# Zilong-Li/BaseVarC

Hardware: AMD Instinct MI355X
Metric: sites/sec at N=1e6 samples; achieved HBM GB/s vs roofline (higher is better)
Workload: dtype f64

## Files before the change

basevarc_amd/csrc/bvc_context.hip:

```cpp
#include <cmath>
#include <cstdlib>
#include <cstring>
#include <mutex>
#include <new>

#include "bvc_ctx.h"

hipError_t sync_streams(bvc_ctx *ctx)
{
    hipError_t first = hipSuccess;
    for (hipStream_t s : streams_of(ctx)) {
        const hipError_t e = hipStreamSynchronize(s);
        if (first == hipSuccess) first = e;
    }
    for (bool &p : ctx->em_pending) p = false;
    return first;
}

int drain_on_error(bvc_ctx *ctx, int code)
{
    (void)sync_streams(ctx);
    (void)hipGetLastError();
    return code;
}
// ... 71 lines not shown
namespace {
std::mutex g_pinned_mu;
std::vector<std::pair<const char *, size_t>> g_pinned;
}

bool in_pinned(const void *p, size_t n)
{
    std::lock_guard<std::mutex> g(g_pinned_mu);
    const char *c = static_cast<const char *>(p);
    for (auto const &r : g_pinned)
        if (c >= r.first && c + n <= r.first + r.second) return true;
    return false;
}

namespace {
struct Knob {
    const char *key, *env;
    int lo, hi, step, dflt;
    int LaunchState::*member;
    bool takes(int v) const { return v >= lo && v <= hi && (v - lo) % step == 0; }
};
const Knob kKnobs[] = {
    {"em_waves_per_cu", "BVC_EM_WAVES_PER_CU", 0, 32, 1, 0, &LaunchState::em_waves_per_cu},
    {"em_wpb", "BVC_EM_WPB", 1, 4, 3, 4, &LaunchState::em_wpb},
    {"hist_split", "BVC_HIST_SPLIT", 0, 64, 1, 0, &LaunchState::hist_split},
    {"group_pipe", "BVC_GROUP_PIPE", 0, 1, 1, 1, &LaunchState::group_pipe},
    {"group_copies_log2", "BVC_GROUP_LOG2C", -1, 5, 1, -1, &LaunchState::group_log2c},
    {"group_big_lds", "BVC_GROUP_BIG_LDS", 0, 1, 1, 1, &LaunchState::group_big_lds},
    {"group_h16", "BVC_GROUP_H16", 0, 1, 1, 0, &LaunchState::group_h16},
    {"em_streams", "BVC_EM_STREAMS", 0, 3, 1, 0, &LaunchState::em_streams},
    {"em_engine", "BVC_EM_ENGINE", 0, 1, 1, 0, &LaunchState::em_engine},
    {"em_tiny_regions", "BVC_EM_TINY_REGIONS", 0, 1, 1, 0, &LaunchState::em_tiny_regions},
    {"em_prune", "BVC_EM_PRUNE", 0, 1, 1, 1, &LaunchState::em_prune},
    {"bgzf_codes", "BVC_BGZF_CODES", 0, 1, 1, 0, &LaunchState::bgzf_codes},
    {"bgzf_parse", "BVC_BGZF_PARSE", 0, 1, 1, 0, &LaunchState::bgzf_parse},
    {"bgzf_cuts", "BVC_BGZF_CUTS", 0, 1, 1, 0, &LaunchState::bgzf_cuts},
    {"csr_scatter_max", "BVC_CSR_SCATTER_MAX", 0, 1 << 30, 1, 64, &LaunchState::csr_scatter_max},
    {"stats_copies_log2", "BVC_STATS_LOG2C", 0, kStatsMaxLog2c, 1, 2, &LaunchState::stats_log2c},
    {"host_chunk_kib", nullptr, 1, 1 << 21, 1, 1 << 19, &LaunchState::host_chunk_kib},
};
}

extern "C" {

const char *bvc_version(void) { return "libbvc 0.3.0 (gfx950)"; }

int bvc_device_count(void)
{
    int n = 0;
    if (hipGetDeviceCount(&n) != hipSuccess) { (void)hipGetLastError(); return 0; }
    int ok = 0;
    for (int d = 0; d < n; ++d) {
        hipDeviceProp_t p;
        if (hipGetDeviceProperties(&p, d) == hipSuccess && std::strncmp(p.gcnArchName, "gfx950", 6) == 0) ++ok;
    }
    return ok;
}

static int env_int(const char *name, int lo, int hi, int dflt)
{
    const char *e = getenv(name);
    if (!e) return dflt;
    const int v = atoi(e);
    return (v >= lo && v <= hi) ? v : dflt;
}

// ... 241 lines not shown
```

basevarc_amd/csrc/bvc_internal.h:

```cpp
#pragma once
#include <hip/hip_runtime.h>
#include <stdint.h>

#include <vector>

#include "../../include/bvc.h"

struct bvc_bam_site_tally;

namespace bvc {

struct LaunchState {
    int n_cu = 256;
    int em_waves_per_cu = 0;
    int em_wpb = 4;
    int hist_split = 0;
    int host_chunk_kib = 1 << 19;
    int em_streams = 0;
    int group_pipe = 1;
    int group_log2c = -1;
    int group_big_lds = 1;
    int group_h16 = 0;
    int em_engine = 0;
    int em_tiny_regions = 0;
    int csr_scatter_max = 64;
    int em_prune = 1;
    int stats_log2c = 2;
    int bgzf_codes = 0;
    int bgzf_parse = 0;
    int bgzf_cuts = 0;
    int dbg_levels = 0;
    mutable uint32_t em_epoch = 0;
    struct RaisedLds { const void *kernel; size_t bytes; };
    mutable std::vector<RaisedLds> lds_raised;
};

inline size_t round256(size_t n) { return (n + 255) / 256 * 256; }

struct Layout {
    uintptr_t base = 0;
    size_t at = 0;
    template <class T> T *take(size_t count, size_t pad = 0)
    {
        T *p = reinterpret_cast<T *>(base + at);
        at += round256(count * sizeof(T) + pad);
        return p;
    }
};

hipError_t raise_lds(const LaunchState &st, const void *kernel, size_t bytes);

struct QualLut {
    double a[128];
    double e[128];
    double e_empty;
    double log_e[128];
    double log_a[128];
};

hipError_t launch_hist_dense(LaunchState &st, hipStream_t stream, int64_t n_sites, int64_t n_samples, int64_t row_stride,
                             const int8_t *bases, const int8_t *quals, const uint8_t *group_of_sample,
                             int n_groups, uint32_t *counts, int split, int64_t *group_scratch = nullptr,
                             uint8_t *hist_of_sample = nullptr);
constexpr int kGroupScratchWords = BVC_MAX_GROUPS + 4;
inline size_t group_redo_offset(int64_t n_samples) { return ((size_t)n_samples + 255) & ~(size_t)255; }
inline size_t group_labels_bytes(int64_t n_samples, int64_t n_sites) { return group_redo_offset(n_samples) + (size_t)n_sites + 256; }
int choose_hist_split(const LaunchState &st, int64_t n_sites, int64_t n_samples);

hipError_t launch_hist_packed(LaunchState &st, hipStream_t stream, int64_t n_sites, int64_t n_samples, int64_t row_stride,
                              const uint8_t *packed, uint32_t *counts, int split);
hipError_t launch_hist_packed_groups(LaunchState &st, hipStream_t stream, int64_t n_sites, int64_t n_samples,
                                     int64_t row_stride, const uint8_t *packed, const uint8_t *group_of_sample, int n_groups,
                                     uint32_t *counts, int64_t *group_scratch, uint8_t *hist_of_sample);
hipError_t launch_pack_dense(hipStream_t stream, int64_t n_sites, int64_t n_samples, int64_t stride_in, const int8_t *bases,
                             const int8_t *quals, int64_t stride_out, uint8_t *packed, unsigned long long *bad);

hipError_t launch_stream_read(hipStream_t stream, const void *src, int64_t bytes, uint32_t *sink);

hipError_t launch_hist_csr(LaunchState &st, hipStream_t stream, int64_t n_sites, const int64_t *offsets,
                           const int8_t *bases, const int8_t *quals, uint32_t *counts);

inline bool uses_item_engine(const LaunchState &st, double min_af) { return st.em_engine != 1 && min_af > 0.0; }
hipError_t launch_lrt(const LaunchState &st, hipStream_t stream, int64_t n_sites, const uint32_t *counts,
                      int64_t hist_stride, const int8_t *ref_base, double min_af, const QualLut *lut,
                      const int8_t *comb, const uint8_t *n_comb, bvc_site_result *results, bool shared = false,
                      int shared_waves_per_cu = 0,
                      void *scratch = nullptr);

size_t em_items_scratch_bytes(int64_t n_sites);
hipError_t launch_lrt_items(const LaunchState &st, hipStream_t stream, int64_t n_sites, int n_groups,
                            const uint32_t *counts, int64_t hist_stride, const int8_t *ref_base, double min_af,
                            const QualLut *lut, const int8_t *comb, const uint8_t *n_comb, bvc_site_result *results,
                            void *scratch, const uint8_t **taken_out, bool shared = false);

hipError_t launch_lrt_groups(const LaunchState &st, hipStream_t stream, int64_t n_sites, int n_groups,
                             const uint32_t *grp_counts, const int8_t *ref_base, double min_af, const QualLut *lut,
                             const bvc_site_result *overall, bvc_group_result *grp_results, bool shared = false,
                             int shared_waves_per_cu = 0, void *scratch = nullptr);
size_t em_group_scratch_bytes(int64_t n_sites, int n_groups);
constexpr int kGroupSharedWavesPerCu = 8;

hipError_t launch_sum_groups(hipStream_t stream, int64_t n_sites, int n_hist, const uint32_t *grp_counts,
                             uint32_t *counts);

hipError_t launch_synth_dense(hipStream_t stream, uint64_t seed, int64_t site0, int64_t n_sites,
                              int64_t n_samples, int64_t row_stride, uint32_t cov_thr16,
                              int8_t *bases, int8_t *quals, int8_t *ref_base);

struct PileupTile {
    const uint8_t *text = nullptr;
    bool bin = false;
    const uint32_t *line_start = nullptr;
    const int32_t *sample0 = nullptr, *n_in_batch = nullptr;
    int32_t n_batches = 0, n_pos = 0;
    int32_t line_stride = 0;
    const int32_t *n_pos_dev = nullptr;
    int64_t n_lines_cap = 0;
    uint32_t *line_words = nullptr;
    uint32_t *status = nullptr;
    int64_t *entry_off = nullptr, *obs_off = nullptr, *totals = nullptr;
    bvc_pileup_entry *entries = nullptr;
    int32_t *samples = nullptr;
    int8_t *obs_base = nullptr, *obs_qual = nullptr;
    const uint8_t *group_of_sample = nullptr;
    int64_t n_samples = 0;
    int32_t n_groups = 0;
    uint8_t *obs_label = nullptr;
    int32_t *tally = nullptr;
    bvc_pileup_indel *indels = nullptr;
    uint32_t indel_cap = 0;
};
struct bvc_pileup_region { uint32_t start, len, left_src, left_len; };
hipError_t launch_region_carry(hipStream_t stream, const uint8_t *old_text, uint8_t *text, const bvc_pileup_region *regions, int32_t n_batches);
hipError_t launch_region_index(hipStream_t stream, const PileupTile &P, const bvc_pileup_region *regions, const uint32_t *seg_base,
                               int64_t n_segments, uint32_t *seg_nl, int32_t *lines, int32_t max_pos);
hipError_t launch_region_ends(hipStream_t stream, const PileupTile &P, uint32_t *ends);
// ... 126 lines not shown
```

basevarc_amd/csrc/bvc_lrt.hip:

```cpp
#include "bvc_ctx.h"

namespace {

int em_stream_count(const bvc_ctx *ctx, int by_default) { return ctx->ls.em_streams > 0 ? ctx->ls.em_streams : by_default; }

hipStream_t em_stream(bvc_ctx *ctx, int by_default)
{
    const int n = em_stream_count(ctx, by_default);
    const int k = (int)(ctx->side_flip++ % (unsigned)n);
    return k == 0 ? ctx->side : (k == 1 ? ctx->side_b : ctx->side_c);
}

int em_scratch_for(bvc_ctx *ctx, int slot, int64_t n_sites, double min_af, void **out, int n_groups = 0)
{
    *out = nullptr;
    if (!uses_item_engine(ctx->ls, min_af)) return BVC_OK;
    const size_t need = n_groups > 0 ? em_group_scratch_bytes(n_sites, n_groups) : em_items_scratch_bytes(n_sites);
    DevBuf &buf = n_groups > 0 ? ctx->d_emg[slot] : ctx->d_em[slot];
    const int rc = ensure_joined(ctx, buf, need);
    if (rc != BVC_OK) return rc;
    *out = buf.p;
    return BVC_OK;
}

// ... 144 lines not shown
        if (rc != BVC_OK) return rc;
        if (n_rows == 1) d.rows[1] = d.rows[0];
    }
    return run_chunks(ctx, n_sites, chunk,
        [&](int set, int64_t s0, int64_t ns) -> int {
            const DenseSet &d = sets[set];
            const size_t bytes = n_samples ? (size_t)(ns - 1) * (size_t)row_stride + (size_t)n_samples : 0;
            if (n_groups > 0 && s0 < 2 * chunk && n_samples)
                BVC_HIP(ctx, hipMemcpyAsync(d.labels, labels, (size_t)n_samples, hipMemcpyHostToDevice, ctx->copy));
            for (int a = 0; a < n_rows && bytes; ++a)
                BVC_HIP(ctx, hipMemcpyAsync(d.rows[a], rows[a] + s0 * row_stride, bytes, hipMemcpyHostToDevice, ctx->copy));
            BVC_HIP(ctx, hipMemcpyAsync(d.ref, ref_base + s0, (size_t)ns, hipMemcpyHostToDevice, ctx->copy));
            return BVC_OK;
        },
        [&](int set, int64_t s0, int64_t ns, bool download) -> int {
            const DenseSet &d = sets[set];
            if (!download) {
                int rc = device(ns, d);
                return rc == BVC_OK ? join_side(ctx) : rc;
            }
            BVC_HIP(ctx, hipMemcpyAsync(results + s0, d.res, (size_t)ns * sizeof(bvc_site_result), hipMemcpyDeviceToHost, ctx->stream));
            if (n_groups > 0)
                BVC_HIP(ctx, hipMemcpyAsync(grp_results + s0 * n_groups, d.gres, (size_t)ns * n_groups * sizeof(bvc_group_result),
                                            hipMemcpyDeviceToHost, ctx->stream));
            return BVC_OK;
        });
}

template <class Stage1>
int run_group_stages(bvc_ctx *ctx, int64_t ns, int n_groups, bool long_rows, Stage1 stage1, const int8_t *r, double min_af,
                     bvc_site_result *res, bvc_group_result *gres, const uint32_t *grp_in = nullptr)
{
    return run_stages(ctx, ns, n_groups, false, min_af, 2, stage1, [&](hipStream_t s2, const RingSlot &slot) -> int {
        BVC_HIP(ctx, launch_sum_groups(s2, ns, n_groups + 1, slot.grp, slot.counts));
        const bool shared = ctx->overlap && long_rows;
        const int per_launch = kGroupSharedWavesPerCu / em_stream_count(ctx, 2) > 2 ? kGroupSharedWavesPerCu / em_stream_count(ctx, 2) : 2;
        BVC_HIP(ctx, launch_lrt(ctx->ls, s2, ns, slot.counts, BVC_NCLASS, r, min_af, ctx->d_lut, nullptr, nullptr, res, shared, per_launch,
                                slot.em));
        BVC_HIP(ctx, launch_lrt_groups(ctx->ls, s2, ns, n_groups, slot.grp, r, min_af, ctx->d_lut, res, gres, shared, per_launch, slot.emg));
        return BVC_OK;
    }, grp_in);
}

int run_csr_groups_device(bvc_ctx *ctx, int64_t n_sites, const int64_t *offsets, const int8_t *bases, const int8_t *quals,
                          const int32_t *sample_of_obs, const int8_t *ref_base, double min_af, const uint8_t *group_of_sample,
                          int64_t n_samples, int32_t n_groups, bvc_site_result *results, bvc_group_result *grp_results)
{
    return run_group_stages(ctx, n_sites, n_groups, false,
                            [&](uint32_t *gp) {
                                return launch_hist_csr_groups(ctx->ls, ctx->stream, n_sites, offsets, bases, quals, sample_of_obs,
                                                              group_of_sample, n_samples, n_groups, gp);
                            },
                            ref_base, min_af, results, grp_results);
}


struct ObsArray { const void *host; size_t elem; void *dev; };

template <class Device>
int run_csr_groups_host(bvc_ctx *ctx, int64_t n_sites, const int64_t *offsets, const int8_t *ref_base, const uint8_t *group_of_sample,
                        int64_t n_samples, ObsArray *arrays, int n_arrays, int32_t n_groups, bvc_site_result *results,
                        bvc_group_result *grp_results, Device device)
{
    const size_t total = (size_t)offsets[n_sites];
    int64_t *d_o; int8_t *d_r; uint8_t *d_g; bvc_site_result *d_res; bvc_group_result *d_gres;
    int rc = carve(ctx, ctx->d_stage[0], 256, [&](Layout &L) {
        d_o = L.take<int64_t>((size_t)n_sites + 1);
// ... 476 lines not shown
```

basevarc_amd/csrc/em_items.hip:

```cpp
#include <algorithm>

#include "bvc_device.h"
#include "bvc_internal.h"
#include "em_common.h"

namespace bvc {
namespace {



constexpr int kTiny = 8, kNarrow = 32, kWide = 48;
template <int CPB> constexpr int site_table_bytes() { return 4 * CPB * 5; }

constexpr int kEmptyQ = 128;

struct FitItem {
    int32_t site;
    uint8_t base[4];
    double f0[4];
    double e_excl;
    double inv_n;
    double ll_excl;
};
static_assert(sizeof(FitItem) == 64, "FitItem layout");
// ... 690 lines not shown
        finished = true;
    }
    S.sets = sets; S.n_emit = (int8_t)n_emit; S.p_deepest = (int8_t)p_deepest;
    int want[kLists];
    count_wanted(sets, n_emit, want);
    if (lane == 0) {
        if (finished) {
            store_record(results + site, S, (int)ref_base[ref_index(site, n_groups)], S.n, S.blist);
            S.state = 2;
        }
        R.site[ls] = S;
        R.want[ls][0] = want[0]; R.want[ls][1] = want[1];
    }
}

struct RegionArgs {
    int64_t n_sites;
    int n_groups;
    const uint32_t *counts;
    int64_t hist_stride;
    const QualLut *lut;
    const int8_t *ref_base;
    double min_af;
    const int8_t *comb;
    const uint8_t *n_comb;
    uint8_t *taken;
    bvc_site_result *results;
    uint32_t *kind_epoch;
    uint32_t epoch;
    int dbg_levels;
    int tiny_regions;
    int prune;
    int64_t region0;
};

__device__ __forceinline__ void wave_sync()
{
    __builtin_amdgcn_fence(__ATOMIC_RELEASE, "workgroup");
    __builtin_amdgcn_wave_barrier();
    __builtin_amdgcn_fence(__ATOMIC_ACQUIRE, "workgroup");
}

__device__ __forceinline__ void load_counts(uint32_t (&c)[8], const uint32_t *__restrict__ counts, int64_t hist_stride, int64_t site,
                                            int n_groups, int lane)
{
    const uint32_t *hist = counts + hist_index(site, n_groups) * hist_stride + (lane >> 4) * 128 + (lane & 15);
#pragma unroll
    for (int lvl = 0; lvl < 8; ++lvl) c[lvl] = hist[16 * lvl];
}

template <int TEAM, class RegionT>
__device__ __forceinline__ void team_sync(RegionT &R, uint32_t &phase, int lane)
{
    if (TEAM == 1) { wave_sync(); return; }
    __builtin_amdgcn_fence(__ATOMIC_RELEASE, "workgroup");
    __builtin_amdgcn_wave_barrier();
    phase += TEAM;
    if (lane == 0) {
        __hip_atomic_fetch_add(&R.arrive, 1u, __ATOMIC_RELEASE, __HIP_MEMORY_SCOPE_WORKGROUP);
        while (__hip_atomic_load(&R.arrive, __ATOMIC_ACQUIRE, __HIP_MEMORY_SCOPE_WORKGROUP) - phase > 0x7FFFFFFFu) __builtin_amdgcn_s_sleep(1);
    }
    __builtin_amdgcn_wave_barrier();
    __builtin_amdgcn_fence(__ATOMIC_ACQUIRE, "workgroup");
}

template <int CPB, int TEAM>
__device__ __forceinline__ void region_body(Region<CPB> *regions, const RegionArgs &A)
{
    const int wave = __builtin_amdgcn_readfirstlane((int)(threadIdx.x >> 6));
    const int teams = (int)(blockDim.x >> 6) / TEAM;
    const int member = wave % TEAM;
    const int lane = threadIdx.x & (kWave - 1);
    Region<CPB> &R = regions[wave / TEAM];
    const int64_t n_sites = A.n_sites;
    const int64_t n_regions = (n_sites + kRegionSites - 1) / kRegionSites;
    if (CPB == kWide && A.kind_epoch[1] != A.epoch) return;
    if (CPB == kTiny && A.kind_epoch[0] != A.epoch) return;
    uint32_t phase = 0;
    if (TEAM > 1) {
        if (member == 0 && lane == 0) R.arrive = 0u;
        __syncthreads();
    }
    const int64_t region = A.region0 + (int64_t)blockIdx.x * teams + wave / TEAM;
    for (bool first = true; region < n_regions && first; first = false) {
        const int64_t site0 = region * kRegionSites;
        if (member == 0 && lane == 0) { R.need = 0; R.next_slot = 0; }
        if (TEAM > 1) team_sync<TEAM>(R, phase, lane);
        int need = 0;
        uint32_t cnext[8];
        if (site0 + member < n_sites) load_counts(cnext, A.counts, A.hist_stride, site0 + member, A.n_groups, lane);
#pragma unroll 1
        for (int ls = member; ls < kRegionSites; ls += TEAM) {
            uint32_t c8[8];
#pragma unroll
            for (int k = 0; k < 8; ++k) c8[k] = cnext[k];
            if (ls + TEAM < kRegionSites && site0 + ls + TEAM < n_sites) load_counts(cnext, A.counts, A.hist_stride, site0 + ls + TEAM, A.n_groups, lane);
            if (site0 + ls < n_sites) {
                need = max(need, site_classes<CPB>(R, ls, lane, site0 + ls, c8, A.lut, A.min_af, A.comb, A.n_comb, A.taken));
            } else if (lane == 0) {
                R.site[ls].state = 2; R.site[ls].n_emit = 0;
                R.want[ls][0] = 0; R.want[ls][1] = 0;
            }
        }
        if (TEAM > 1) {
            if (lane == 0) atomicMax(&R.need, need);
            team_sync<TEAM>(R, phase, lane);
            need = R.need;
        } else {
            wave_sync();
        }
        const int kind = (A.tiny_regions && need <= kTiny) ? kTiny : (need <= kNarrow ? kNarrow : kWide);
        if (CPB == kNarrow && kind != kNarrow && member == 0 && lane == 0) A.kind_epoch[kind == kWide ? 1 : 0] = A.epoch;
        if (kind != CPB) {
            if (TEAM > 1) team_sync<TEAM>(R, phase, lane);
            continue;
        }
        if (member == 0 && lane < kRegionSites && R.site[lane].state == 3) {
            const int64_t site = site0 + lane;
            store_record(A.results + site, R.site[lane], (int)A.ref_base[ref_index(site, A.n_groups)], R.site[lane].n,
                         R.site[lane].blist);
            R.site[lane].state = 2;
        }
        team_sync<TEAM>(R, phase, lane);
        for (int round = 0; round < kRounds && round < (A.dbg_levels >> 1); ++round) {
            int cnt[kLists] = {0, 0};
#pragma unroll
            for (int w = 0; w < kRegionSites; ++w) {
#pragma unroll
                for (int l = 0; l < kLists; ++l) cnt[l] += R.want[w][l];
// ... 24 lines not shown
            team_sync<TEAM>(R, phase, lane);
            if (TEAM > 1 && member == 0 && lane == 0) R.next_slot = 0;
            if (round + 1 == (A.dbg_levels >> 1) && (A.dbg_levels & 1)) break;
            int my = lane;
            asm volatile("" : "+v"(my));
            if (member == 0 && my < kRegionSites && site0 + my < n_sites)
                site_decide(R, my, 0, site0 + my, A.n_groups, A.prune, A.ref_base, A.results);
            team_sync<TEAM>(R, phase, lane);
        }
        team_sync<TEAM>(R, phase, lane);
    }
}

#define BVC_OCCUPANCY(n) BVC_WAVES_PER_EU(n, n)
#ifdef BVC_RCP_CHUNK
#define BVC_REGION_WAVES_PER_EU 4
#else
#define BVC_REGION_WAVES_PER_EU 3
#endif
constexpr int kMaxRegionWaves = 4;
#ifndef BVC_REGION_TEAM
#define BVC_REGION_TEAM 2
#endif
constexpr int kTeam = BVC_REGION_TEAM;

template <int CPB>
__global__ __launch_bounds__(64 * kMaxRegionWaves) BVC_OCCUPANCY(CPB == kWide ? 2 : BVC_REGION_WAVES_PER_EU) void region_kernel(RegionArgs A)
{
    BVC_POISON_LDS();
    extern __shared__ __attribute__((aligned(16))) unsigned char region_lds[];
    region_body<CPB, kTeam>(reinterpret_cast<Region<CPB> *>(region_lds), A);
}

}

#ifdef BVC_CHECK_LDS
BVC_DEFINE_DEBUG_READER(debug_read_items)
#endif

struct ItemScratch {
    uint8_t *taken;
    uint32_t *kind_epoch;
};

static ItemScratch item_scratch(Layout &L, int64_t n_sites)
{
    const size_t start = L.at;
    ItemScratch s;
    s.taken = L.take<uint8_t>((size_t)n_sites);
    s.kind_epoch = L.take<uint32_t>(0);
    L.at = start + (size_t)n_sites + 256 + 64;
    return s;
}

size_t em_items_scratch_bytes(int64_t n_sites)
{
    Layout size;
    item_scratch(size, n_sites);
    return size.at;
}

hipError_t launch_lrt_items(const LaunchState &st, hipStream_t stream, int64_t n_sites, int n_groups,
                            const uint32_t *counts, int64_t hist_stride, const int8_t *ref_base, double min_af,
                            const QualLut *lut, const int8_t *comb, const uint8_t *n_comb, bvc_site_result *results,
                            void *scratch, const uint8_t **taken_out, bool shared)
{
    Layout slices{reinterpret_cast<uintptr_t>(scratch)};
    const ItemScratch scr = item_scratch(slices, n_sites);
    uint8_t *taken = scr.taken;
    const int64_t regions = (n_sites + kRegionSites - 1) / kRegionSites;
    int per_cu = 0;
    if (st.em_waves_per_cu > 0) per_cu = st.em_waves_per_cu;
    else if (shared) per_cu = 4;
    constexpr int kMaxTeams = kMaxRegionWaves / kTeam;
    int teams;
    int64_t wgs, per_launch;
    if (per_cu > 0) {
        const int want_teams = std::max(1, per_cu / kTeam);
        teams = std::min(want_teams, kMaxTeams);
        wgs = (regions + teams - 1) / teams;
        per_launch = (int64_t)st.n_cu * ((want_teams + teams - 1) / teams);
    } else {
        teams = (int)std::min<int64_t>(kMaxTeams, std::max<int64_t>(1, (regions + st.n_cu - 1) / st.n_cu));
        wgs = (regions + teams - 1) / teams;
        per_launch = wgs;
    }
    RegionArgs A;
    A.n_sites = n_sites; A.n_groups = n_groups; A.counts = counts; A.hist_stride = hist_stride; A.lut = lut;
    A.ref_base = ref_base; A.min_af = min_af; A.comb = comb; A.n_comb = n_comb; A.taken = taken; A.results = results;
    A.kind_epoch = scr.kind_epoch;
    A.epoch = ++st.em_epoch;
    if (A.epoch == 0) A.epoch = ++st.em_epoch;
    A.dbg_levels = st.dbg_levels > 0 ? st.dbg_levels : 2 * kRounds;
    A.tiny_regions = st.em_tiny_regions;
    A.prune = st.em_prune;
    A.region0 = 0;
    const hipError_t e = raise_lds(st, reinterpret_cast<const void *>(region_kernel<kWide>), kMaxTeams * sizeof(Region<kWide>));
    if (e != hipSuccess) return e;
    const dim3 block(64 * teams * kTeam);
    auto sequence = [&](auto kernel, size_t lds_per_team) {
        for (int64_t w0 = 0; w0 < wgs; w0 += per_launch) {
            A.region0 = w0 * teams;
            hipLaunchKernelGGL(kernel, dim3((unsigned)std::min(per_launch, wgs - w0)), block, teams * lds_per_team, stream, A);
        }
        A.region0 = 0;
    };
    sequence(region_kernel<kNarrow>, sizeof(Region<kNarrow>));
    if (st.em_tiny_regions) sequence(region_kernel<kTiny>, sizeof(Region<kTiny>));
    sequence(region_kernel<kWide>, sizeof(Region<kWide>));
    *taken_out = taken;
    return hipGetLastError();
}

}
```

basevarc_amd/csrc/em_kernel.hip:

```cpp
#include "bvc_device.h"
#include "bvc_internal.h"
#include "em_common.h"

namespace bvc {
namespace {

template <int NS>
struct Slots {
    double n[NS];
    double e[NS];
    double d[NS];
    double yp[NS];
};

struct Freq {
    double fb;
};

constexpr int kDppRor8 = 0x128;
constexpr int kDppRowBcast15 = 0x142;
template <int L> constexpr int dpp_newbcast() { return 0x150 + L; }

struct PassOut {
    double ex_own;
    bool converged;
};


template <int NS, int NA = NS>
__device__ __forceinline__ PassOut em_pass(Slots<NS> &S, const Freq f, double inv_n, int lane)
{
    static_assert(NA >= 1 && NA <= NS, "active slots");
// ... 376 lines not shown
            bvc_group_result r;
            for (int j = 0; j < 4; ++j) r.depth[j] = o.depth[j];
            for (int j = 0; j < 6; ++j) r.pad[j] = 0;
            r.ran = o.depth_total > 0 ? 1 : 0;
            r.present = 0;
#pragma unroll
            for (int i = 0; i < 3; ++i) {
                double af = 0.0;
                if (r.ran && i < ov.n_alt) {
#pragma unroll
                    for (int tt = 0; tt < 3; ++tt)
                        if (tt < o.n_alt && o.alt_base[tt] == ov.alt_base[i]) { af = o.af[tt]; r.present |= (uint8_t)(1u << i); }
                }
                r.af[i] = af;
            }
            grp_results[site * n_groups + g] = r;
        }
        wave_lds_sync<WPB>();
    }
}

__global__ void var_qual_kernel(int64_t n_sites, bvc_site_result *__restrict__ results)
{
    BVC_POISON_LDS();
    const int64_t s = (int64_t)blockIdx.x * blockDim.x + threadIdx.x;
    if (s >= n_sites) return;
    if (!results[s].called || results[s].var_qual != kVarQualPending) return;
    const double p = kf_gammaq_dev(0.5, results[s].chi / 2.0);
    double vq = (p != 0.0) ? -10 * log10(p) : 10000.0;
    if (vq == 0) vq = 0.0;
    results[s].var_qual = vq;
}

__global__ void sum_groups_kernel(int64_t total, int n_hist, const uint32_t *__restrict__ grp_counts,
                                  uint32_t *__restrict__ counts)
{
    BVC_POISON_LDS();
    const int64_t i = (int64_t)blockIdx.x * blockDim.x + threadIdx.x;
    if (i >= total) return;
    const int64_t site = i / BVC_NCLASS;
    const int key = (int)(i % BVC_NCLASS);
    uint32_t s = 0;
    for (int h = 0; h < n_hist; ++h) s += grp_counts[(site * n_hist + h) * BVC_NCLASS + key];
    counts[i] = s;
}

__global__ void group_comb_kernel(int64_t n_pseudo, int n_groups, const int8_t *__restrict__ ref_base,
                                  const bvc_site_result *__restrict__ overall, int8_t *__restrict__ comb,
                                  uint8_t *__restrict__ n_comb)
{
    BVC_POISON_LDS();
    const int64_t p = (int64_t)blockIdx.x * blockDim.x + threadIdx.x;
    if (p >= n_pseudo) return;
    const int64_t site = p / n_groups;
    int nc = 0;
    int8_t list[4] = {0, 0, 0, 0};
    if (overall[site].called) {
        const int ref = ref_base[site];
        if ((unsigned)ref < 4u) list[nc++] = (int8_t)ref;
        const int n_alt = overall[site].n_alt;
        for (int i = 0; i < 3; ++i)
            if (i < n_alt) list[nc++] = (int8_t)(overall[site].alt_base[i] & 3);
    }
    for (int c = 0; c < 4; ++c) comb[p * 4 + c] = list[c];
    n_comb[p] = (uint8_t)nc;
}

__global__ void group_records_kernel(int64_t n_pseudo, int n_groups, const bvc_site_result *__restrict__ overall,
                                     const bvc_site_result *__restrict__ pseudo, const uint8_t *__restrict__ taken,
                                     bvc_group_result *__restrict__ grp_results)
{
    BVC_POISON_LDS();
    const int64_t p = (int64_t)blockIdx.x * blockDim.x + threadIdx.x;
    if (p >= n_pseudo || !taken[p]) return;
    const int64_t site = p / n_groups;
    const bvc_site_result t = pseudo[p];
    bvc_group_result r;
    for (int j = 0; j < 4; ++j) r.depth[j] = t.depth[j];
    for (int j = 0; j < 6; ++j) r.pad[j] = 0;
    for (int j = 0; j < 3; ++j) r.af[j] = 0.0;
    r.ran = 0; r.present = 0;
    if (overall[site].called) {
        r.ran = t.depth_total > 0 ? 1 : 0;
        const int n_alt = overall[site].n_alt;
        for (int i = 0; i < 3; ++i)
            if (r.ran && i < n_alt)
                for (int tt = 0; tt < 3; ++tt)
                    if (tt < t.n_alt && t.alt_base[tt] == overall[site].alt_base[i]) { r.af[i] = t.af[tt]; r.present |= (uint8_t)(1u << i); }
    }
    grp_results[p] = r;
}

}

#ifdef BVC_CHECK_LDS
BVC_DEFINE_DEBUG_READER(debug_read_wave_engine)
#endif


static int64_t em_grid_cap(const LaunchState &st, bool shared, int shared_waves_per_cu = 0)
{
    int per_cu = shared ? (shared_waves_per_cu > 0 ? shared_waves_per_cu : 8) : 24;
    if (st.em_waves_per_cu > 0) per_cu = st.em_waves_per_cu;
    return (int64_t)per_cu * st.n_cu;
}

struct SiteKernels {
    template <int NS, int WPB, bool ANY = false> static constexpr auto kernel() { return lrt_kernel<NS, WPB, ANY>; }
};
struct GroupKernels {
    template <int NS, int WPB, bool ANY = false> static constexpr auto kernel() { return lrt_groups_kernel<NS, WPB, ANY>; }
};

template <class Family, int WPB, class... Args>
static void launch_variants(hipStream_t stream, int64_t want_waves, const uint8_t *taken, Args... args)
{
    const dim3 grid((unsigned)((want_waves + WPB - 1) / WPB)), block(64 * WPB);
    if (taken) {
        hipLaunchKernelGGL((Family::template kernel<8, WPB, true>()), grid, block, 0, stream, args...);
        return;
    }
    hipLaunchKernelGGL((Family::template kernel<2, WPB>()), grid, block, 0, stream, args...);
    hipLaunchKernelGGL((Family::template kernel<4, WPB>()), grid, block, 0, stream, args...);
// ... 8 lines not shown
    const int64_t want_waves = n_work < cap ? n_work : cap;
    if (st.em_wpb == 1) launch_variants<Family, 1>(stream, want_waves, taken, args...);
    else launch_variants<Family, 4>(stream, want_waves, taken, args...);
}

template <class Kernel, class... Args>
static void launch_per_element(Kernel kernel, hipStream_t stream, int64_t n, Args... args)
{
    hipLaunchKernelGGL(kernel, dim3((unsigned)((n + 255) / 256)), dim3(256), 0, stream, n, args...);
}

hipError_t launch_lrt(const LaunchState &st, hipStream_t stream, int64_t n_sites, const uint32_t *counts,
                      int64_t hist_stride, const int8_t *ref_base, double min_af, const QualLut *lut,
                      const int8_t *comb, const uint8_t *n_comb, bvc_site_result *results, bool shared,
                      int shared_waves_per_cu, void *scratch)
{
    if (n_sites <= 0) return hipSuccess;
    const uint8_t *taken = nullptr;
    if (scratch && uses_item_engine(st, min_af)) {
        const hipError_t e = launch_lrt_items(st, stream, n_sites, 0, counts, hist_stride, ref_base, min_af, lut, comb, n_comb,
                                              results, scratch, &taken, shared);
        if (e != hipSuccess) return e;
    }
    launch_wave_kernels<SiteKernels>(st, stream, n_sites, shared, shared_waves_per_cu, taken, n_sites, counts, hist_stride, ref_base,
                                     min_af, lut, comb, n_comb, taken, results);
    launch_per_element(var_qual_kernel, stream, n_sites, results);
    return hipGetLastError();
}

struct GroupScratch {
    int8_t *comb;
    uint8_t *n_comb;
    bvc_site_result *pseudo;
    void *items;
};

static GroupScratch group_scratch(Layout &L, int64_t n_pseudo)
{
    GroupScratch s;
    s.comb = L.take<int8_t>((size_t)n_pseudo * 4);
    s.n_comb = L.take<uint8_t>((size_t)n_pseudo);
    s.pseudo = L.take<bvc_site_result>((size_t)n_pseudo);
    s.items = L.take<char>(0);
    L.at += em_items_scratch_bytes(n_pseudo);
    return s;
}

size_t em_group_scratch_bytes(int64_t n_sites, int n_groups)
{
    Layout size;
    group_scratch(size, n_sites * n_groups);
    return size.at;
}

hipError_t launch_lrt_groups(const LaunchState &st, hipStream_t stream, int64_t n_sites, int n_groups,
                             const uint32_t *grp_counts, const int8_t *ref_base, double min_af, const QualLut *lut,
                             const bvc_site_result *overall, bvc_group_result *grp_results, bool shared,
                             int shared_waves_per_cu, void *scratch)
{
    if (n_sites <= 0 || n_groups <= 0) return hipSuccess;
    const int64_t n_work = n_sites * n_groups;
    const uint8_t *taken = nullptr;
    if (scratch && uses_item_engine(st, min_af)) {
        Layout slices{reinterpret_cast<uintptr_t>(scratch)};
        const GroupScratch s = group_scratch(slices, n_work);
        launch_per_element(group_comb_kernel, stream, n_work, n_groups, ref_base, overall, s.comb, s.n_comb);
        const hipError_t e = launch_lrt_items(st, stream, n_work, n_groups, grp_counts, BVC_NCLASS, ref_base, min_af, lut, s.comb,
                                              s.n_comb, s.pseudo, s.items, &taken, shared);
        if (e != hipSuccess) return e;
        launch_per_element(group_records_kernel, stream, n_work, n_groups, overall, s.pseudo, taken, grp_results);
    }
    launch_wave_kernels<GroupKernels>(st, stream, n_work, shared, shared_waves_per_cu, taken, n_sites, n_groups, grp_counts, ref_base,
                                      min_af, lut, overall, taken, grp_results);
    return hipGetLastError();
}

hipError_t launch_sum_groups(hipStream_t stream, int64_t n_sites, int n_hist, const uint32_t *grp_counts,
                             uint32_t *counts)
{
    const int64_t total = n_sites * BVC_NCLASS;
    if (total <= 0) return hipSuccess;
    launch_per_element(sum_groups_kernel, stream, total, n_hist, grp_counts, counts);
    return hipGetLastError();
}

}
```

Baseline: 3.358 million.

## Compact live group pseudo-sites before EM and fill dead ones directly

```diff
diff --git a/basevarc_amd/csrc/bvc_context.hip b/basevarc_amd/csrc/bvc_context.hip
--- a/basevarc_amd/csrc/bvc_context.hip
+++ b/basevarc_amd/csrc/bvc_context.hip
@@ -127,6 +127,7 @@
     {"em_engine", "BVC_EM_ENGINE", 0, 1, 1, 0, &LaunchState::em_engine},
     {"em_tiny_regions", "BVC_EM_TINY_REGIONS", 0, 1, 1, 0, &LaunchState::em_tiny_regions},
     {"em_prune", "BVC_EM_PRUNE", 0, 1, 1, 1, &LaunchState::em_prune},
+    {"group_live", "BVC_GROUP_LIVE", 0, 1, 1, 1, &LaunchState::group_live},
     {"bgzf_codes", "BVC_BGZF_CODES", 0, 1, 1, 0, &LaunchState::bgzf_codes},
     {"bgzf_parse", "BVC_BGZF_PARSE", 0, 1, 1, 0, &LaunchState::bgzf_parse},
     {"bgzf_cuts", "BVC_BGZF_CUTS", 0, 1, 1, 0, &LaunchState::bgzf_cuts},
diff --git a/basevarc_amd/csrc/bvc_internal.h b/basevarc_amd/csrc/bvc_internal.h
--- a/basevarc_amd/csrc/bvc_internal.h
+++ b/basevarc_amd/csrc/bvc_internal.h
@@ -25,6 +25,7 @@
     int em_tiny_regions = 0;
     int csr_scatter_max = 64;
     int em_prune = 1;
+    int group_live = 1;
     int stats_log2c = 2;
     int bgzf_codes = 0;
     int bgzf_parse = 0;
@@ -91,7 +92,8 @@
 hipError_t launch_lrt_items(const LaunchState &st, hipStream_t stream, int64_t n_sites, int n_groups,
                             const uint32_t *counts, int64_t hist_stride, const int8_t *ref_base, double min_af,
                             const QualLut *lut, const int8_t *comb, const uint8_t *n_comb, bvc_site_result *results,
-                            void *scratch, const uint8_t **taken_out, bool shared = false);
+                            void *scratch, const uint8_t **taken_out, bool shared = false, const uint32_t *n_live = nullptr,
+                            const int32_t *rows = nullptr);
 
 hipError_t launch_lrt_groups(const LaunchState &st, hipStream_t stream, int64_t n_sites, int n_groups,
                              const uint32_t *grp_counts, const int8_t *ref_base, double min_af, const QualLut *lut,
@@ -101,7 +103,8 @@
 constexpr int kGroupSharedWavesPerCu = 8;
 
 hipError_t launch_sum_groups(hipStream_t stream, int64_t n_sites, int n_hist, const uint32_t *grp_counts,
-                             uint32_t *counts);
+                             uint32_t *counts, void *live_scratch = nullptr);
+void *group_live_scratch(const LaunchState &st, double min_af, void *group_scratch_buf);
 
 hipError_t launch_synth_dense(hipStream_t stream, uint64_t seed, int64_t site0, int64_t n_sites,
                               int64_t n_samples, int64_t row_stride, uint32_t cov_thr16,
diff --git a/basevarc_amd/csrc/bvc_lrt.hip b/basevarc_amd/csrc/bvc_lrt.hip
--- a/basevarc_amd/csrc/bvc_lrt.hip
+++ b/basevarc_amd/csrc/bvc_lrt.hip
@@ -200,7 +200,7 @@
                      bvc_site_result *res, bvc_group_result *gres, const uint32_t *grp_in = nullptr)
 {
     return run_stages(ctx, ns, n_groups, false, min_af, 2, stage1, [&](hipStream_t s2, const RingSlot &slot) -> int {
-        BVC_HIP(ctx, launch_sum_groups(s2, ns, n_groups + 1, slot.grp, slot.counts));
+        BVC_HIP(ctx, launch_sum_groups(s2, ns, n_groups + 1, slot.grp, slot.counts, group_live_scratch(ctx->ls, min_af, slot.emg)));
         const bool shared = ctx->overlap && long_rows;
         const int per_launch = kGroupSharedWavesPerCu / em_stream_count(ctx, 2) > 2 ? kGroupSharedWavesPerCu / em_stream_count(ctx, 2) : 2;
         BVC_HIP(ctx, launch_lrt(ctx->ls, s2, ns, slot.counts, BVC_NCLASS, r, min_af, ctx->d_lut, nullptr, nullptr, res, shared, per_launch,
diff --git a/basevarc_amd/csrc/em_items.hip b/basevarc_amd/csrc/em_items.hip
--- a/basevarc_amd/csrc/em_items.hip
+++ b/basevarc_amd/csrc/em_items.hip
@@ -746,6 +746,8 @@
     int tiny_regions;
     int prune;
     int64_t region0;
+    const uint32_t *n_live;
+    const int32_t *rows;
 };
 
 __device__ __forceinline__ void wave_sync()
@@ -778,7 +780,7 @@
     __builtin_amdgcn_fence(__ATOMIC_ACQUIRE, "workgroup");
 }
 
-template <int CPB, int TEAM>
+template <int CPB, int TEAM, bool LIVE = false>
 __device__ __forceinline__ void region_body(Region<CPB> *regions, const RegionArgs &A)
 {
     const int wave = __builtin_amdgcn_readfirstlane((int)(threadIdx.x >> 6));
@@ -786,10 +788,15 @@
     const int member = wave % TEAM;
     const int lane = threadIdx.x & (kWave - 1);
     Region<CPB> &R = regions[wave / TEAM];
-    const int64_t n_sites = A.n_sites;
+    int64_t n_sites = A.n_sites;
+    if constexpr (LIVE) n_sites = (int64_t)*A.n_live;
     const int64_t n_regions = (n_sites + kRegionSites - 1) / kRegionSites;
     if (CPB == kWide && A.kind_epoch[1] != A.epoch) return;
     if (CPB == kTiny && A.kind_epoch[0] != A.epoch) return;
+    auto row_of = [&](int64_t site) -> int64_t {
+        if constexpr (LIVE) return (int64_t)A.rows[site];
+        else return site;
+    };
     uint32_t phase = 0;
     if (TEAM > 1) {
         if (member == 0 && lane == 0) R.arrive = 0u;
@@ -802,13 +809,13 @@
         if (TEAM > 1) team_sync<TEAM>(R, phase, lane);
         int need = 0;
         uint32_t cnext[8];
-        if (site0 + member < n_sites) load_counts(cnext, A.counts, A.hist_stride, site0 + member, A.n_groups, lane);
+        if (site0 + member < n_sites) load_counts(cnext, A.counts, A.hist_stride, row_of(site0 + member), A.n_groups, lane);
 #pragma unroll 1
         for (int ls = member; ls < kRegionSites; ls += TEAM) {
             uint32_t c8[8];
 #pragma unroll
             for (int k = 0; k < 8; ++k) c8[k] = cnext[k];
-            if (ls + TEAM < kRegionSites && site0 + ls + TEAM < n_sites) load_counts(cnext, A.counts, A.hist_stride, site0 + ls + TEAM, A.n_groups, lane);
+            if (ls + TEAM < kRegionSites && site0 + ls + TEAM < n_sites) load_counts(cnext, A.counts, A.hist_stride, row_of(site0 + ls + TEAM), A.n_groups, lane);
             if (site0 + ls < n_sites) {
                 need = max(need, site_classes<CPB>(R, ls, lane, site0 + ls, c8, A.lut, A.min_af, A.comb, A.n_comb, A.taken));
             } else if (lane == 0) {
@@ -899,6 +906,14 @@
     region_body<CPB, kTeam>(reinterpret_cast<Region<CPB> *>(region_lds), A);
 }
 
+template <int CPB>
+__global__ __launch_bounds__(64 * kMaxRegionWaves) BVC_OCCUPANCY(CPB == kWide ? 2 : BVC_REGION_WAVES_PER_EU) void region_live_kernel(RegionArgs A)
+{
+    BVC_POISON_LDS();
+    extern __shared__ __attribute__((aligned(16))) unsigned char region_lds[];
+    region_body<CPB, kTeam, true>(reinterpret_cast<Region<CPB> *>(region_lds), A);
+}
+
 }
 
 #ifdef BVC_CHECK_LDS
@@ -930,7 +945,7 @@
 hipError_t launch_lrt_items(const LaunchState &st, hipStream_t stream, int64_t n_sites, int n_groups,
                             const uint32_t *counts, int64_t hist_stride, const int8_t *ref_base, double min_af,
                             const QualLut *lut, const int8_t *comb, const uint8_t *n_comb, bvc_site_result *results,
-                            void *scratch, const uint8_t **taken_out, bool shared)
+                            void *scratch, const uint8_t **taken_out, bool shared, const uint32_t *n_live, const int32_t *rows)
 {
     Layout slices{reinterpret_cast<uintptr_t>(scratch)};
     const ItemScratch scr = item_scratch(slices, n_sites);
@@ -962,7 +977,10 @@
     A.tiny_regions = st.em_tiny_regions;
     A.prune = st.em_prune;
     A.region0 = 0;
-    const hipError_t e = raise_lds(st, reinterpret_cast<const void *>(region_kernel<kWide>), kMaxTeams * sizeof(Region<kWide>));
+    A.n_live = n_live; A.rows = rows;
+    const bool live = n_live != nullptr;
+    const hipError_t e = raise_lds(st, live ? reinterpret_cast<const void *>(region_live_kernel<kWide>) : reinterpret_cast<const void *>(region_kernel<kWide>),
+                                   kMaxTeams * sizeof(Region<kWide>));
     if (e != hipSuccess) return e;
     const dim3 block(64 * teams * kTeam);
     auto sequence = [&](auto kernel, size_t lds_per_team) {
@@ -972,6 +990,13 @@
         }
         A.region0 = 0;
     };
+    if (live) {
+        sequence(region_live_kernel<kNarrow>, sizeof(Region<kNarrow>));
+        if (st.em_tiny_regions) sequence(region_live_kernel<kTiny>, sizeof(Region<kTiny>));
+        sequence(region_live_kernel<kWide>, sizeof(Region<kWide>));
+        *taken_out = taken;
+        return hipGetLastError();
+    }
     sequence(region_kernel<kNarrow>, sizeof(Region<kNarrow>));
     if (st.em_tiny_regions) sequence(region_kernel<kTiny>, sizeof(Region<kTiny>));
     sequence(region_kernel<kWide>, sizeof(Region<kWide>));
diff --git a/basevarc_amd/csrc/em_kernel.hip b/basevarc_amd/csrc/em_kernel.hip
--- a/basevarc_amd/csrc/em_kernel.hip
+++ b/basevarc_amd/csrc/em_kernel.hip
@@ -1,3 +1,5 @@
+#include <algorithm>
+
 #include "bvc_device.h"
 #include "bvc_internal.h"
 #include "em_common.h"
@@ -440,17 +442,39 @@
     results[s].var_qual = vq;
 }
 
-__global__ void sum_groups_kernel(int64_t total, int n_hist, const uint32_t *__restrict__ grp_counts,
-                                  uint32_t *__restrict__ counts)
-{
-    BVC_POISON_LDS();
-    const int64_t i = (int64_t)blockIdx.x * blockDim.x + threadIdx.x;
-    if (i >= total) return;
-    const int64_t site = i / BVC_NCLASS;
-    const int key = (int)(i % BVC_NCLASS);
-    uint32_t s = 0;
-    for (int h = 0; h < n_hist; ++h) s += grp_counts[(site * n_hist + h) * BVC_NCLASS + key];
-    counts[i] = s;
+__global__ __launch_bounds__(BVC_NCLASS) void sum_groups_kernel(int64_t n_sites, int n_hist, const uint32_t *__restrict__ grp_counts,
+                                                                uint32_t *__restrict__ counts, int32_t *__restrict__ depth)
+{
+    BVC_POISON_LDS();
+    __shared__ int32_t part[BVC_MAX_GROUPS][8];
+    const int key = threadIdx.x, lane = key & (kWave - 1);
+    const int wave = __builtin_amdgcn_readfirstlane(key >> 6);
+    const int n_groups = n_hist - 1;
+    for (int64_t site = blockIdx.x; site < n_sites; site += gridDim.x) {
+        const uint32_t *h = grp_counts + site * n_hist * BVC_NCLASS + key;
+        uint32_t s = 0;
+        for (int g0 = 0; g0 < n_hist; g0 += 8) {
+            uint32_t v[8];
+#pragma unroll
+            for (int i = 0; i < 8; ++i) v[i] = g0 + i < n_hist ? h[(int64_t)(g0 + i) * BVC_NCLASS] : 0u;
+#pragma unroll
+            for (int i = 0; i < 8; ++i) {
+                s += v[i];
+                if (depth && g0 + i < n_groups) {
+                    const int d = row_sum((int)v[i]);
+                    const int dw = __builtin_amdgcn_readlane(d, 0) + __builtin_amdgcn_readlane(d, 16) + __builtin_amdgcn_readlane(d, 32) +
+                                   __builtin_amdgcn_readlane(d, 48);
+                    if (lane == 0) part[g0 + i][wave] = dw;
+                }
+            }
+        }
+        counts[site * BVC_NCLASS + key] = s;
+        if (depth) {
+            __syncthreads();
+            if (key < 4 * n_groups) depth[site * n_groups * 4 + key] = part[key >> 2][2 * (key & 3)] + part[key >> 2][2 * (key & 3) + 1];
+            __syncthreads();
+        }
+    }
 }
 
 __global__ void group_comb_kernel(int64_t n_pseudo, int n_groups, const int8_t *__restrict__ ref_base,
@@ -474,29 +498,122 @@
     n_comb[p] = (uint8_t)nc;
 }
 
-__global__ void group_records_kernel(int64_t n_pseudo, int n_groups, const bvc_site_result *__restrict__ overall,
-                                     const bvc_site_result *__restrict__ pseudo, const uint8_t *__restrict__ taken,
-                                     bvc_group_result *__restrict__ grp_results)
+__global__ void group_live_kernel(int64_t n_pseudo, int n_groups, const bvc_site_result *__restrict__ overall,
+                                  const int32_t *__restrict__ depth, uint8_t *__restrict__ done,
+                                  bvc_group_result *__restrict__ grp_results)
 {
     BVC_POISON_LDS();
     const int64_t p = (int64_t)blockIdx.x * blockDim.x + threadIdx.x;
-    if (p >= n_pseudo || !taken[p]) return;
+    if (p >= n_pseudo) return;
     const int64_t site = p / n_groups;
-    const bvc_site_result t = pseudo[p];
+    const int d0 = depth[p * 4], d1 = depth[p * 4 + 1], d2 = depth[p * 4 + 2], d3 = depth[p * 4 + 3];
+    const bool live = overall[site].called && d0 + d1 + d2 + d3 > 0;
+    if (!live) grp_results[p] = group_record_depths(d0, d1, d2, d3);
+    done[p] = live ? 0 : 1;
+}
+
+constexpr int kScanThreads = 1024, kScanPerThread = 16;
+__global__ __launch_bounds__(kScanThreads) void group_scan_kernel(int64_t n_pseudo, const uint8_t *__restrict__ done,
+                                                                  int32_t *__restrict__ order, uint32_t *__restrict__ n_live)
+{
+    BVC_POISON_LDS();
+    __shared__ uint32_t wave_sum[kScanThreads / kWave];
+    __shared__ uint32_t running;
+    const int lane = threadIdx.x & (kWave - 1), wave = threadIdx.x >> 6;
+    if (threadIdx.x == 0) running = 0;
+    __syncthreads();
+    for (int64_t t0 = 0; t0 < n_pseudo; t0 += (int64_t)kScanThreads * kScanPerThread) {
+        const int64_t first = t0 + (int64_t)threadIdx.x * kScanPerThread;
+        uint32_t live_bits = 0;
+        if (first < n_pseudo) {
+            const uint4 f = *reinterpret_cast<const uint4 *>(done + first);
+            const uint32_t w[4] = {f.x, f.y, f.z, f.w};
+#pragma unroll
+            for (int i = 0; i < kScanPerThread; ++i)
+                if (first + i < n_pseudo && ((w[i >> 2] >> (8 * (i & 3))) & 0xFFu) == 0) live_bits |= 1u << i;
+        }
+        const uint32_t mine = (uint32_t)__popc(live_bits);
+        uint32_t incl = mine;
+        for (int d = 1; d < kWave; d <<= 1) {
+            const uint32_t up = __shfl_up(incl, d);
+            if (lane >= d) incl += up;
+        }
+        if (lane == kWave - 1) wave_sum[wave] = incl;
+        __syncthreads();
+        uint32_t before = running;
+        for (int w = 0; w < wave; ++w) before += wave_sum[w];
+        uint32_t j = before + incl - mine;
+        for (uint32_t bits = live_bits; bits; bits &= bits - 1) order[j++] = (int32_t)(first + (__ffs(bits) - 1));
+        __syncthreads();
+        if (threadIdx.x == kScanThreads - 1) running = before + incl;
+        __syncthreads();
+    }
+    if (threadIdx.x == 0) *n_live = running;
+}
+
+__global__ void group_pack_kernel(int64_t n_pseudo, int n_groups, const uint32_t *__restrict__ n_live, const int32_t *__restrict__ order,
+                                  const int8_t *__restrict__ ref_base, const bvc_site_result *__restrict__ overall,
+                                  int32_t *__restrict__ rows, int8_t *__restrict__ ref_packed, int8_t *__restrict__ comb,
+                                  uint8_t *__restrict__ n_comb)
+{
+    BVC_POISON_LDS();
+    const int64_t j = (int64_t)blockIdx.x * blockDim.x + threadIdx.x;
+    if (j >= n_pseudo || j >= (int64_t)*n_live) return;
+    const int64_t p = order[j];
+    const int64_t site = p / n_groups;
+    rows[j] = (int32_t)(p + site);
+    const int ref = ref_base[site];
+    ref_packed[j] = (int8_t)ref;
+    int nc = 0;
+    int8_t list[4] = {0, 0, 0, 0};
+    if ((unsigned)ref < 4u) list[nc++] = (int8_t)ref;
+    const int n_alt = overall[site].n_alt;
+    for (int i = 0; i < 3; ++i)
+        if (i < n_alt) list[nc++] = (int8_t)(overall[site].alt_base[i] & 3);
+    for (int c = 0; c < 4; ++c) comb[j * 4 + c] = list[c];
+    n_comb[j] = (uint8_t)nc;
+}
+
+__device__ __forceinline__ bvc_group_result group_record_of(const bvc_site_result &t, const bvc_site_result &ov)
+{
     bvc_group_result r;
     for (int j = 0; j < 4; ++j) r.depth[j] = t.depth[j];
     for (int j = 0; j < 6; ++j) r.pad[j] = 0;
     for (int j = 0; j < 3; ++j) r.af[j] = 0.0;
     r.ran = 0; r.present = 0;
-    if (overall[site].called) {
+    if (ov.called) {
         r.ran = t.depth_total > 0 ? 1 : 0;
-        const int n_alt = overall[site].n_alt;
+        const int n_alt = ov.n_alt;
         for (int i = 0; i < 3; ++i)
             if (r.ran && i < n_alt)
                 for (int tt = 0; tt < 3; ++tt)
-                    if (tt < t.n_alt && t.alt_base[tt] == overall[site].alt_base[i]) { r.af[i] = t.af[tt]; r.present |= (uint8_t)(1u << i); }
-    }
-    grp_results[p] = r;
+                    if (tt < t.n_alt && t.alt_base[tt] == ov.alt_base[i]) { r.af[i] = t.af[tt]; r.present |= (uint8_t)(1u << i); }
+    }
+    return r;
+}
+
+__global__ void group_records_kernel(int64_t n_pseudo, int n_groups, const bvc_site_result *__restrict__ overall,
+                                     const bvc_site_result *__restrict__ pseudo, const uint8_t *__restrict__ taken,
+                                     bvc_group_result *__restrict__ grp_results)
+{
+    BVC_POISON_LDS();
+    const int64_t p = (int64_t)blockIdx.x * blockDim.x + threadIdx.x;
+    if (p >= n_pseudo || !taken[p]) return;
+    grp_results[p] = group_record_of(pseudo[p], overall[p / n_groups]);
+}
+
+__global__ void group_live_records_kernel(int64_t n_pseudo, int n_groups, const uint32_t *__restrict__ n_live,
+                                          const int32_t *__restrict__ order, const bvc_site_result *__restrict__ overall,
+                                          const bvc_site_result *__restrict__ pseudo, const uint8_t *__restrict__ taken,
+                                          uint8_t *__restrict__ done, bvc_group_result *__restrict__ grp_results)
+{
+    BVC_POISON_LDS();
+    const int64_t j = (int64_t)blockIdx.x * blockDim.x + threadIdx.x;
+    if (j >= n_pseudo || j >= (int64_t)*n_live) return;
+    const int64_t p = order[j];
+    if (!taken[j]) return;
+    done[p] = 1;
+    grp_results[p] = group_record_of(pseudo[j], overall[p / n_groups]);
 }
 
 }
@@ -571,6 +688,11 @@
     int8_t *comb;
     uint8_t *n_comb;
     bvc_site_result *pseudo;
+    int32_t *depth;
+    uint8_t *done;
+    int32_t *order, *rows;
+    int8_t *ref;
+    uint32_t *n_live;
     void *items;
 };
 
@@ -580,6 +702,12 @@
     s.comb = L.take<int8_t>((size_t)n_pseudo * 4);
     s.n_comb = L.take<uint8_t>((size_t)n_pseudo);
     s.pseudo = L.take<bvc_site_result>((size_t)n_pseudo);
+    s.depth = L.take<int32_t>((size_t)n_pseudo * 4);
+    s.done = L.take<uint8_t>((size_t)n_pseudo);
+    s.order = L.take<int32_t>((size_t)n_pseudo);
+    s.rows = L.take<int32_t>((size_t)n_pseudo);
+    s.ref = L.take<int8_t>((size_t)n_pseudo);
+    s.n_live = L.take<uint32_t>(1);
     s.items = L.take<char>(0);
     L.at += em_items_scratch_bytes(n_pseudo);
     return s;
@@ -600,7 +728,20 @@
     if (n_sites <= 0 || n_groups <= 0) return hipSuccess;
     const int64_t n_work = n_sites * n_groups;
     const uint8_t *taken = nullptr;
-    if (scratch && uses_item_engine(st, min_af)) {
+    if (group_live_scratch(st, min_af, scratch)) {
+        Layout slices{reinterpret_cast<uintptr_t>(scratch)};
+        const GroupScratch s = group_scratch(slices, n_work);
+        launch_per_element(group_live_kernel, stream, n_work, n_groups, overall, s.depth, s.done, grp_results);
+        hipLaunchKernelGGL(group_scan_kernel, dim3(1), dim3(kScanThreads), 0, stream, n_work, s.done, s.order, s.n_live);
+        launch_per_element(group_pack_kernel, stream, n_work, n_groups, s.n_live, s.order, ref_base, overall, s.rows, s.ref, s.comb, s.n_comb);
+        const uint8_t *taken_packed = nullptr;
+        const hipError_t e = launch_lrt_items(st, stream, n_work, 0, grp_counts, BVC_NCLASS, s.ref, min_af, lut, s.comb, s.n_comb, s.pseudo,
+                                              s.items, &taken_packed, shared, s.n_live, s.rows);
+        if (e != hipSuccess) return e;
+        launch_per_element(group_live_records_kernel, stream, n_work, n_groups, s.n_live, s.order, overall, s.pseudo, taken_packed, s.done,
+                           grp_results);
+        taken = s.done;
+    } else if (scratch && uses_item_engine(st, min_af)) {
         Layout slices{reinterpret_cast<uintptr_t>(scratch)};
         const GroupScratch s = group_scratch(slices, n_work);
         launch_per_element(group_comb_kernel, stream, n_work, n_groups, ref_base, overall, s.comb, s.n_comb);
@@ -615,12 +756,22 @@
 }
 
 hipError_t launch_sum_groups(hipStream_t stream, int64_t n_sites, int n_hist, const uint32_t *grp_counts,
-                             uint32_t *counts)
-{
-    const int64_t total = n_sites * BVC_NCLASS;
-    if (total <= 0) return hipSuccess;
-    launch_per_element(sum_groups_kernel, stream, total, n_hist, grp_counts, counts);
+                             uint32_t *counts, void *live_scratch)
+{
+    if (n_sites <= 0) return hipSuccess;
+    int32_t *depth = nullptr;
+    if (live_scratch && n_hist > 1) {
+        Layout slices{reinterpret_cast<uintptr_t>(live_scratch)};
+        depth = group_scratch(slices, n_sites * (n_hist - 1)).depth;
+    }
+    hipLaunchKernelGGL(sum_groups_kernel, dim3((unsigned)std::min<int64_t>(n_sites, 1 << 20)), dim3(BVC_NCLASS), 0, stream, n_sites, n_hist,
+                       grp_counts, counts, depth);
     return hipGetLastError();
 }
 
-}
+void *group_live_scratch(const LaunchState &st, double min_af, void *group_scratch_buf)
+{
+    return group_scratch_buf && uses_item_engine(st, min_af) && st.group_live ? group_scratch_buf : nullptr;
+}
+
+}
```

New measurement: 3.342 million. Within noise of the previous version (-0.5%).
